# CGLemon/Sayuri

Measured on AMD Instinct MI355X. Metric: nn_evals_per_sec, higher is better.
Workload: dtype f16

## Files before the change

sayuri_amd/csrc/hip/engine_graph.h:

```cpp
#pragma once
#include "engine_plan.h"

namespace sayuri {

class EngineBase {
public:
    virtual ~EngineBase() {}
    virtual int load_tensor(int layer, int kind, const float* host, size_t n) = 0;
    virtual int upload(int n, const float* planes, const int* board_sizes, const unsigned* packed = nullptr, int binary = 0) = 0;
    virtual int run() = 0;
    virtual int sync() = 0;
    virtual int download(float* prob, float* pass, float* misc, float* own) = 0;
    virtual int time_runs(int iters, float* ms) = 0;
    virtual int profile_run(sayuri_hip_kernel_stat* rows, int cap) = 0;
    virtual int submit(int n, const float* planes, const int* bsz, float* prob, float* pass, float* misc, float* own,
                       int* ticket, const unsigned* packed = nullptr, int binary = 0) = 0;
    virtual int wait(int ticket) = 0;
    virtual int query(int ticket) = 0;
    virtual int mark_kernel(const char* name) = 0;
    virtual int timed_stat(sayuri_hip_kernel_stat* row) = 0;
    virtual size_t device_bytes() const = 0;
    virtual int last_chains() const = 0;
    virtual int tower_state() const = 0;
    virtual int latency_state() const = 0;
// ... 1085 lines not shown
    int rows_use(const Fwd& f, const ConvParams& p, const char* layer) {
        const void* use[3] = {p.in, p.out, p.res};
        for (int u = 0; u < 3 && flags_.dbg_recycle_input < 2; ++u)
            for (int i = 0; i < kNumBufs; ++i) {
                if (!use[u] || f.io.bufs[i] != use[u]) continue;
                const int stride = u ? p.cout_s : p.cin_s;
                if (rows_stride_[i] && rows_stride_[i] != stride)
                    return fail(std::string("activation buffer ") + std::to_string(i) + " is used with row stride " + std::to_string(stride) + " by " +
                                layer + " and with " + std::to_string(rows_stride_[i]) + " by " + (rows_first_[i] ? rows_first_[i] : "?") +
                                " inside one persistent run / chained forward: the rows of different tiles would overlap");
                rows_stride_[i] = stride;
                rows_first_[i] = layer;
            }
        return 0;
    }

    const ConvLayerDev& cv(int id) const { return convs_.at(id); }
    const FcLayerDev& fc(int id) const { return fcs_.at(id); }

    int forward(int t, float* zc_pass = nullptr, float* zc_misc = nullptr) {
        const int G = chains_for_batch();
        last_chains_ = G;
        rows_reset();
        IoSlot& io = io_[t];
        Fwd f{t, io, compute_[t]};
        f.ntiles = plan().ntiles;
        f.ns = geom_.n;
        f.px = geom_.total;
        f.pass = zc_pass ? zc_pass : io.pass;
        f.misc = zc_misc ? zc_misc : io.misc;
        if (sx_kts_) {
            int nse = 0;
            for (const auto& b : blocks_) nse += b.apply_se ? 1 : 0;
            if (io.sx_epoch > 0xfff00000u) {
                HIP_OK(hipMemsetAsync(io.sx_xchg, 0, sizeof(unsigned long long) * (size_t)max_batch_ * sx_kts_ * kSxMaxSub * kSxSlots, f.stream));
                io.sx_epoch = 0;
            }
            f.sx_epoch0 = io.sx_epoch;
            io.sx_epoch += (unsigned)nse;
        }
        if (G <= 1) return forward_graph(f);
        if (chain_setup(G)) return -1;
        const BoardTabs* tabs = nullptr;
        if (board_tabs(f, &tabs)) return -1;
        HIP_OK(hipEventRecord(chain_fork_, f.stream));
        const int nt = board_plan_.ntiles;
        for (int g = 0; g < G; ++g) {
            Fwd c = f;
            c.stream = chain_stream_[g];
            c.chained = true;
            c.tile0 = (int)((long)nt * g / G);
            c.ntiles = (int)((long)nt * (g + 1) / G) - c.tile0;
            c.n0 = board_plan_.tile_first[c.tile0];
            c.ns = board_plan_.tile_first[c.tile0 + c.ntiles] - c.n0;
            c.px = geom_.off[c.n0 + c.ns] - geom_.off[c.n0];
            hipError_t e = hipStreamWaitEvent(c.stream, chain_fork_, 0);
            if (flags_.chains_serial && g > 0 && e == hipSuccess) e = hipStreamWaitEvent(c.stream, chain_join_[g - 1], 0);
            if (e == hipSuccess && forward_graph(c)) return -1;
            if (e == hipSuccess) e = hipEventRecord(chain_join_[g], c.stream);
            if (e != hipSuccess) return fail(std::string("chained forward: ") + hipGetErrorString(e));
        }
        for (int g = 0; g < G; ++g) HIP_OK(hipStreamWaitEvent(f.stream, chain_join_[g], 0));
        return 0;
    }

    int pack_input(Fwd& f, T* dst) {
        const int cin = desc_.input_channels, cs = cv(SAYURI_L_INPUT_CONV).cin_s, board = board_;
        const int n0 = f.n0, ns = f.ns;
        const double px = f.px;
        const BatchGeom g = dgeom(f.io);
        const IoSlot& io = f.io;
        if (io.packed_binary > 0) {
            const unsigned* rec = io.packed_src ? io.packed_src : io.packed;
            const int split = io.packed_src ? 1 : kPackSplit;
            const int nbin = io.packed_binary, words = nbin * 12 + 8;
            return timed(f, "pack_input", 0, (double)ns * words * 4 + px * cs * sizeof(T), [&] {
                hipLaunchKernelGGL(pack_bits_kernel<T>, dim3(ns * split), dim3(256), 0, f.stream, rec, words, nbin, dst, g, cin, cs,
                                   io.g_perm, n0, split);
            });
        }
        const int grid = ns * kPackSplit;
        const int chunk = pack_input_chunk(slot_pix_, cs, (int)sizeof(T));
        const size_t lds = (size_t)chunk * (cs * sizeof(T) + 16);
        const size_t flat_lds = pack_input_flat_lds(slot_pix_, cs, (int)sizeof(T));
        const bool flat = flat_lds <= 64 * 1024 && (size_t)cin * board * board < 65536;
        return timed(f, "pack_input", 0, px * cin * 4 + px * cs * sizeof(T), [&] {
            if (flat)
                hipLaunchKernelGGL(pack_input_flat_kernel<T>, dim3(ns), dim3(kPackFlatThreads), flat_lds, f.stream,
                                   (const float*)io.planes, dst, g, cin, cs, board, io.g_perm, n0);
            else
                hipLaunchKernelGGL(pack_input_kernel<T>, dim3(grid), dim3(kPackThreads), lds, f.stream,
                                   (const float*)io.planes, dst, g, cin, cs, board, io.g_perm, chunk, n0);
        });
    }

    int forward_graph(Fwd& f) {
        const auto& d = desc_;
        const int C = d.residual_channels, csC = round_up(C, 32), act = d.default_act;
        T* const* buf = f.io.bufs;

        int x = f.take();
        const int in = f.take();
        if (pack_input(f, buf[in])) return -1;
        if (conv(f, "conv3x3_input", cv(SAYURI_L_INPUT_CONV), buf[in], buf[x], nullptr, act)) return -1;
        if (flags_.dbg_recycle_input) f.give(in);

        for (int b = 0; b < d.residual_blocks; ++b) {
            const auto& bd = blocks_[b];
            const bool se = bd.apply_se != 0;
            const int last_act = se ? (int)kIdentity : act;
            const int y = f.take();
            int skip = x;
            bool se_done = false;
            if (bd.type == SAYURI_BLOCK_RESIDUAL) {
                const int t0 = f.take();
                if (conv(f, "conv3x3_tower", cv(SAYURI_L_BLOCK(b, SAYURI_S_CONV1)), buf[x], buf[t0], nullptr, act)) return -1;
                int fused = 1;
                if (se) {
                    fused = conv_se(f, cv(SAYURI_L_BLOCK(b, SAYURI_S_CONV2)), fc(SAYURI_L_BLOCK(b, SAYURI_S_SQUEEZE)),
                                    fc(SAYURI_L_BLOCK(b, SAYURI_S_EXCITE)), buf[t0], buf[y], buf[x], C, act);
                    if (fused == 1)
                        fused = conv_sx(f, cv(SAYURI_L_BLOCK(b, SAYURI_S_CONV2)), fc(SAYURI_L_BLOCK(b, SAYURI_S_SQUEEZE)),
                                        fc(SAYURI_L_BLOCK(b, SAYURI_S_EXCITE)), buf[t0], buf[y], buf[x], C, act);
                    if (fused < 0) return -1;
                    se_done = fused == 0;
                }
                if (fused == 1 &&
                    conv(f, "conv3x3_tower", cv(SAYURI_L_BLOCK(b, SAYURI_S_CONV2)), buf[t0], buf[y], se ? nullptr : buf[x], last_act))
                    return -1;
                f.give(t0);
            } else if (bd.type == SAYURI_BLOCK_BOTTLENECK) {
                const int t0 = f.take(), t1 = f.take();
                if (conv(f, "conv1x1_tower", cv(SAYURI_L_BLOCK(b, SAYURI_S_PRE_BTL)), buf[x], buf[t0], nullptr, act)) return -1;
                if (conv(f, "conv3x3_tower", cv(SAYURI_L_BLOCK(b, SAYURI_S_CONV1)), buf[t0], buf[t1], nullptr, act)) return -1;
                if (conv(f, "conv3x3_tower", cv(SAYURI_L_BLOCK(b, SAYURI_S_CONV2)), buf[t1], buf[t0], nullptr, act)) return -1;
                if (conv(f, "conv1x1_tower", cv(SAYURI_L_BLOCK(b, SAYURI_S_POST_BTL)), buf[t0], buf[y], se ? nullptr : buf[x], last_act)) return -1;
                f.give(t0); f.give(t1);
            } else if (bd.type == SAYURI_BLOCK_NESTED_BOTTLENECK) {
                const int r1 = f.take(), t0 = f.take(), t1 = f.take();
                if (conv(f, "conv1x1_tower", cv(SAYURI_L_BLOCK(b, SAYURI_S_PRE_BTL)), buf[x], buf[r1], nullptr, act)) return -1;
                if (conv(f, "conv3x3_tower", cv(SAYURI_L_BLOCK(b, SAYURI_S_CONV1)), buf[r1], buf[t0], nullptr, act)) return -1;
                if (conv(f, "conv3x3_tower", cv(SAYURI_L_BLOCK(b, SAYURI_S_CONV2)), buf[t0], buf[t1], buf[r1], act)) return -1;
                if (conv(f, "conv3x3_tower", cv(SAYURI_L_BLOCK(b, SAYURI_S_CONV3)), buf[t1], buf[t0], nullptr, act)) return -1;
                if (conv(f, "conv3x3_tower", cv(SAYURI_L_BLOCK(b, SAYURI_S_CONV4)), buf[t0], buf[r1], buf[t1], act)) return -1;
                if (conv(f, "conv1x1_tower", cv(SAYURI_L_BLOCK(b, SAYURI_S_POST_BTL)), buf[r1], buf[y], se ? nullptr : buf[x], last_act)) return -1;
                f.give(r1); f.give(t0); f.give(t1);
            } else {
                const int s2 = f.take(), t1 = f.take();
                if (depthwise(f, "depthwise", cv(SAYURI_L_BLOCK(b, SAYURI_S_DW_CONV)), buf[x], buf[s2], buf[x], act)) return -1;
                if (conv(f, "conv1x1_tower", cv(SAYURI_L_BLOCK(b, SAYURI_S_CONV1)), buf[s2], buf[t1], nullptr, act)) return -1;
                if (conv(f, "conv1x1_tower", cv(SAYURI_L_BLOCK(b, SAYURI_S_CONV2)), buf[t1], buf[y], se ? nullptr : buf[s2], last_act)) return -1;
                f.give(t1);
                f.give(x);
                x = s2;
                skip = s2;
            }
            if (se && !se_done) {
                if (se_unit(f, fc(SAYURI_L_BLOCK(b, SAYURI_S_SQUEEZE)), fc(SAYURI_L_BLOCK(b, SAYURI_S_EXCITE)), buf[y], buf[skip], C, csC,
                            act, f.n0, f.ns))
                    return -1;
            }
            f.give(x);
            x = y;
        }
        return heads(f, x);
    }

    int heads(Fwd& f, int x) {
        const auto& d = desc_;
        const int C = d.residual_channels, csC = round_up(C, 32), act = d.default_act;
        const int Cp = d.policy_head_channels, Cv = d.value_head_channels;
        T* const* buf = f.io.bufs;
// ... 198 lines not shown
```

sayuri_amd/csrc/hip/engine_plan.h:

```cpp
#pragma once
namespace sayuri {

static thread_local std::string g_err;
static std::atomic<unsigned> g_host_free_gen{0};
static thread_local int g_test_conv_kind = 0;
static int fail(const std::string& m) { g_err = m; return -1; }

#define HIP_OK(expr)                                                                      \
    do {                                                                                  \
        hipError_t e_ = (expr);                                                           \
        if (e_ != hipSuccess) {                                                           \
            g_err = std::string(#expr) + ": " + hipGetErrorString(e_);                    \
            return -1;                                                                    \
        }                                                                                 \
    } while (0)

static inline int round_up(int v, int m) { return (v + m - 1) / m * m; }
constexpr size_t kMaxLds = 160 * 1024;
constexpr int kNumCU = 256;

template <typename T> struct ConvKernelTable {
    typedef void (*Fn)(const ConvParams);
    struct Entry { int wmt, wnt; Fn fn; size_t (*lds)(int); int npos_cap; };
    static std::vector<Entry>& entries() {
// ... 28 lines not shown
struct GldsEntry {
    int wmt, wnt;
    void (*fn)(const GldsParams);
    void (*setup)(BatchGeom, int*, int2*);
    size_t lds;
    int npos_cap, npos, pt;
};
static std::vector<GldsEntry>& glds_entries() {
    static std::vector<GldsEntry> e;
    return e;
}
template <int WMT, int WNT> static void register_glds() {
    typedef GldsCfg<WMT, WNT> Cfg;
    glds_entries().push_back({WMT, WNT, &conv_glds_kernel<WMT, WNT>, &tile_setup_kernel<Cfg::PT, Cfg::NPOS>, Cfg::lds_bytes(),
                              Cfg::NPOS_CAP, Cfg::NPOS, Cfg::PT});
}
static void register_all_glds() {
    if (!glds_entries().empty()) return;
    register_glds<8, 3>(); register_glds<8, 2>(); register_glds<8, 1>();
    register_glds<4, 3>(); register_glds<4, 2>(); register_glds<4, 1>();
}
template <typename T> static std::vector<T> board_row_order(const std::vector<T>& img, int ko_pad, int row = 8) {
    std::vector<T> out(img.size());
    const size_t planes = img.size() / ((size_t)ko_pad * row);
    for (size_t pl = 0; pl < planes; ++pl)
        for (int r = 0; r < ko_pad; ++r)
            std::copy_n(img.begin() + (pl * ko_pad + board_row_channel(r)) * row, row, out.begin() + (pl * ko_pad + r) * row);
    return out;
}
static bool board_uses_row_order(int kot) { return (kot / 64) % 2 == 0; }
typedef void (*BoardFn)(const BoardParams);
typedef void (*BoardSeFn)(const BoardSeParams);
struct BoardEntry { int kot; BoardFn fn; BoardSeFn fn_se; size_t (*lds)(int); };
static const BoardEntry kBoardEntries[] = {
    {256, &conv_board_kernel<4>, &conv_board_se_kernel<4>, &BoardCfg<4>::lds_bytes},
    {192, &conv_board_kernel<3>, nullptr, &BoardCfg<3>::lds_bytes},
    {128, &conv_board_kernel<2>, &conv_board_se_kernel<2>, &BoardCfg<2>::lds_bytes},
};
typedef void (*SplitFn)(const SplitParams);
struct SplitEntry { int nj; SplitFn fn; };
static const SplitEntry kSplitEntries[] = {
    {1, &conv_split_kernel<1>}, {2, &conv_split_kernel<2>}, {3, &conv_split_kernel<3>}, {6, &conv_split_kernel<6>}, {12, &conv_split_kernel<12>},
};
typedef void (*HeadFn)(const HeadBoardParams);
struct HeadEntry { int rt, depth; HeadFn fn; };
static const HeadEntry kHeadEntries[] = {
    {2, 5, &head_board_kernel<2, 5>}, {4, 5, &head_board_kernel<4, 5>}, {4, 3, &head_board_kernel<4, 3>},
    {6, 3, &head_board_kernel<6, 3>}, {6, 2, &head_board_kernel<6, 2>},
};
static void enable_big_lds_glds() {
    register_all_glds();
    for (const auto& e : glds_entries())
        (void)hipFuncSetAttribute((const void*)e.fn, hipFuncAttributeMaxDynamicSharedMemorySize, (int)kMaxLds);
    (void)hipFuncSetAttribute((const void*)&conv_board_kernel<4, true>, hipFuncAttributeMaxDynamicSharedMemorySize, (int)kMaxLds);
    for (const auto& e : kHeadEntries) (void)hipFuncSetAttribute((const void*)e.fn, hipFuncAttributeMaxDynamicSharedMemorySize, (int)kMaxLds);
    (void)hipFuncSetAttribute((const void*)&conv_board_sx_kernel<2>, hipFuncAttributeMaxDynamicSharedMemorySize, (int)kMaxLds);
    for (const auto& e : kSplitEntries) (void)hipFuncSetAttribute((const void*)e.fn, hipFuncAttributeMaxDynamicSharedMemorySize, (int)kMaxLds);
    for (const auto& e : kBoardEntries) {
        (void)hipFuncSetAttribute((const void*)e.fn, hipFuncAttributeMaxDynamicSharedMemorySize, (int)kMaxLds);
        if (e.fn_se) (void)hipFuncSetAttribute((const void*)e.fn_se, hipFuncAttributeMaxDynamicSharedMemorySize, (int)kMaxLds);
    }
}
struct ConvOverride {
    bool v0 = false, no_board = false;
    int wnt = 0;
};
struct EngineFlags {
    ConvOverride conv;
    bool tower = true, se_fused = true, heads_fused = true, arith = true;
    bool latency = false;
    int latency_split = 0;
    bool tower_chain = true;
    bool tower_gen_epi = true;
    bool se_split = true;
    int tower_noepi_after = -1;
    unsigned dbg_sx_epoch0 = 0;
    bool dbg_sx_stall = false;
    int sx_dbg = 0;
    int dbg_recycle_input = 0;
    int chains = 0;
    bool chains_serial = false;
    bool tower_sync = false;
    bool fwdstat = false;
    int board_kot = 0;
    int act_override = -1;
    int board_dbg = 0, heads_dbg = 0;
    static bool off(const char* name) { const char* e = getenv(name); return e && atoi(e) == 0; }
    static EngineFlags from_env() {
        EngineFlags f;
        if (const char* e = getenv("SAYURI_CONV")) {
            if (!strncmp(e, "v0", 2)) { f.conv.v0 = true; f.conv.no_board = true; }
            else if (!strncmp(e, "glds", 4)) { f.conv.no_board = true; (void)sscanf(e, "glds:%d", &f.conv.wnt); }
        }
        f.tower = !off("SAYURI_TOWER");
        f.tower_chain = !off("SAYURI_TOWER_CHAIN");
        f.tower_gen_epi = !off("SAYURI_TOWER_GEN_EPI");
        if (const char* e = getenv("SAYURI_DEBUG_RECYCLE_INPUT")) f.dbg_recycle_input = atoi(e);
        f.se_split = !off("SAYURI_SE_SPLIT");
        if (const char* e = getenv("SAYURI_SX_DBG")) f.sx_dbg = atoi(e);
        f.dbg_sx_stall = getenv("SAYURI_DEBUG_SX_STALL") != nullptr;
        if (const char* e = getenv("SAYURI_DEBUG_SX_EPOCH0")) f.dbg_sx_epoch0 = (unsigned)strtoul(e, nullptr, 0);
        if (const char* e = getenv("SAYURI_TOWER_NOEPI_AFTER")) f.tower_noepi_after = atoi(e);
        f.se_fused = !off("SAYURI_SE_FUSED");
        f.heads_fused = !off("SAYURI_HEADS_FUSED");
        f.arith = !getenv("SAYURI_NO_ARITH");
        if (const char* e = getenv("SAYURI_CHAINS")) f.chains = std::max(0, std::min(atoi(e), 4));
        f.chains_serial = getenv("SAYURI_CHAINS_SERIAL") != nullptr;
        f.tower_sync = getenv("SAYURI_TOWER_SYNC") != nullptr;
        f.fwdstat = getenv("SAYURI_HIP_FWDSTAT") != nullptr;
        if (const char* e = getenv("SAYURI_LATENCY_SPLIT")) f.latency_split = std::max(0, atoi(e));
#ifdef SAYURI_EXPERIMENTS
        if (const char* e = getenv("SAYURI_BOARD_KOT")) f.board_kot = atoi(e);
        if (const char* e = getenv("SAYURI_ACT_OVERRIDE")) f.act_override = atoi(e);
        if (const char* e = getenv("SAYURI_BOARD_DBG")) f.board_dbg = atoi(e);
        if (getenv("SAYURI_HEADS_DBG")) f.heads_dbg = 1;
        if (f.board_dbg || f.heads_dbg || f.act_override >= 0) f.tower = false;
#endif
        return f;
    }
    EngineFlags for_latency() const {
        EngineFlags f = *this;
        f.latency = true;
        f.tower = false; f.se_fused = false; f.se_split = false; f.chains = 1;
        return f;
    }
};

template <typename T> static void enable_big_lds() {
    register_all_convs<T>();
    for (const auto& e : ConvKernelTable<T>::entries())
        (void)hipFuncSetAttribute((const void*)e.fn, hipFuncAttributeMaxDynamicSharedMemorySize, (int)kMaxLds);
}

static int pick_wmt(int cout_s, bool fp16) {
    const int opts16[] = {1, 2, 3, 4, 6, 8};
    const int opts32[] = {1, 2, 3, 4};
    const int* opts = fp16 ? opts16 : opts32;
    const int nopts = fp16 ? 6 : 4;
    for (int i = 0; i < nopts; ++i)
        if (opts[i] * 32 >= cout_s) return opts[i];
    int best = opts[nopts - 1], best_pad = 1 << 30;
    for (int i = nopts - 1; i >= 0; --i) {
        const int kot = opts[i] * 32, pad = round_up(cout_s, kot) - cout_s;
        if (pad < best_pad) { best_pad = pad; best = opts[i]; }
    }
    return best;
}

struct HostGeom {
    std::vector<int> bsz, off;
    int n = 0, total = 0;
    void tile_bounds(int PT, int* npos_out, int* nsub_out) const {
        int max_pos = 0, max_sub = 0;
        int s = 0;
        for (int g0 = 0; g0 < total; g0 += PT) {
            const int g1 = std::min(g0 + PT, total);
            while (s + 1 < n && off[s + 1] <= g0) ++s;
            int pos = 0, sub = 0;
            for (int m = s; m < n && off[m] < g1; ++m) {
                const int bs = bsz[m];
                const int a = std::max(g0, off[m]) - off[m], b = std::min(g1, off[m + 1]) - off[m];
                const int rows = (b - 1) / bs - a / bs + 3;
                pos += rows * (bs + 2);
                ++sub;
            }
            max_pos = std::max(max_pos, pos);
            max_sub = std::max(max_sub, sub);
        }
        *npos_out = round_up(std::max(max_pos, 16), 16);
        *nsub_out = max_sub;
    }
};

static bool tile_fits(const HostGeom& geom, int PT, int npos_cap, int* npos) {
    int nsub;
    geom.tile_bounds(PT, npos, &nsub);
    return *npos <= npos_cap && nsub <= kMaxSub;
}
static double tile_cost(const HostGeom& geom, int PT, int kot_tiles, int* ntiles) {
    *ntiles = (geom.total + PT - 1) / PT;
    return std::ceil((double)*ntiles * kot_tiles / kNumCU) * (PT + 24);
}
template <typename T> struct TileChoice { int wnt, npos, ntiles; const typename ConvKernelTable<T>::Entry* e; };
template <typename T> static bool pick_tile(const HostGeom& geom, int wmt, int kot_tiles, bool widest, TileChoice<T>* out) {
    double best = 0;
    out->e = nullptr;
    for (const auto& e : ConvKernelTable<T>::entries()) {
        int npos, ntiles;
        if (e.wmt != wmt || !tile_fits(geom, 64 * e.wnt, e.npos_cap, &npos) || e.lds(npos) > kMaxLds) continue;
        const double cost = tile_cost(geom, 64 * e.wnt, kot_tiles, &ntiles), score = widest ? -e.wnt : cost;
        if (!out->e || score < best) { best = score; *out = TileChoice<T>{e.wnt, npos, ntiles, &e}; }
    }
// ... 383 lines not shown
```

sayuri_amd/csrc/hip/head_board.h:

```cpp
#pragma once
#include "common.h"
#include "conv_board.h"
#include "small_ops.h"

namespace sayuri {

constexpr int kHeadPix = 384;

struct HeadBoardParams {
    const void* trunk;
    const void* w;
    const void* w2;
    const float* bias;
    BatchGeom g;
    int cs;
    int PT, VT;
    HeadParams h;
    unsigned long long* dbg;
    int n0;
};

__host__ __device__ inline int head_vec_floats(int rows) { return 7 * rows + 16 + (16 * rows > 1024 ? 16 * rows : 1024); }
__host__ inline bool head_board_fits(int rows, int nchunks, int depth) {
    return (size_t)nchunks * 4 * rows * 16 + (size_t)depth * 4 * kHeadPix * 16 + sizeof(float) * head_vec_floats(rows) <= 160 * 1024;
}

__device__ __forceinline__ int split_fc(const FcDev fc, const float* x, float* red, int t, int nt) {
    const int parts = max(1, min(nt / fc.out, (fc.in + 7) / 8));
    const int per = (fc.in + parts - 1) / parts;
    for (int idx = t; idx < parts * fc.out; idx += nt) {
        const int o = idx % fc.out, part = idx / fc.out;
        const int i0 = part * per, i1 = min(fc.in, i0 + per);
        const float* w = fc.wt + o;
        float a = 0.f;
        for (int i = i0; i < i1; i += 8) {
            float wv[8];
#pragma unroll
            for (int u = 0; u < 8; ++u) wv[u] = i + u < i1 ? w[(size_t)(i + u) * fc.out] : 0.f;
#pragma unroll
            for (int u = 0; u < 8; ++u) a += (i + u < i1 ? x[i + u] : 0.f) * wv[u];
        }
        red[idx] = a;
    }
    return parts;
}
__device__ __forceinline__ void fold_fc(const FcDev fc, const float* red, int parts, float* y, int act, int t, int nt) {
    for (int o = t; o < fc.out; o += nt) {
        float a = fc.b[o];
        for (int k = 0; k < parts; ++k) a += red[k * fc.out + o];
        y[o] = activate(a, act);
    }
}

template <int RT, int ACT>
__device__ __forceinline__ void head_board_tail(const HeadBoardParams& hp, unsigned char* smem, f32x4 (&acc)[RT][3], const f16x8 (&a2)[RT / 2],
                                                int wave, int lane, int n, int bs, unsigned long long* dbg) {
    constexpr int ROWS = RT * 16;
    const HeadParams& h = hp.h;
    const int tid = wave * 64 + lane, q = lane >> 4, px = lane & 15;
    const int npix = bs * bs, B2 = h.board * h.board;
    const int on_ = h.perm ? h.perm[n] : n;
    float* vec = (float*)(smem + 160 * 1024) - head_vec_floats(ROWS);
    float* pool = vec;
    float* inter = pool + 3 * ROWS;
    float* pinter = inter + 3 * ROWS;
    float* rb = pinter + ROWS;
    float* red = rb + 16;

#pragma unroll
    for (int i = 0; i < RT; ++i)
#pragma unroll
        for (int j = 0; j < 3; ++j) {
            if constexpr (ACT == kMish) {
                const f32x2 lo = mish2(f32x2{acc[i][j][0], acc[i][j][1]}), hi = mish2(f32x2{acc[i][j][2], acc[i][j][3]});
                acc[i][j] = f32x4{lo[0], lo[1], hi[0], hi[1]};
            } else {
#pragma unroll
                for (int r = 0; r < 4; ++r) acc[i][j][r] = activate(acc[i][j][r], ACT);
            }
        }
    f32x4 d[3];
#pragma unroll
    for (int j = 0; j < 3; ++j) {
        d[j] = f32x4{0.f, 0.f, 0.f, 0.f};
#pragma unroll
        for (int t = 0; t < RT / 2; ++t) {
            f16x8 b;
#pragma unroll
            for (int r = 0; r < 4; ++r) { b[r] = (f16)acc[2 * t][j][r]; b[4 + r] = (f16)acc[2 * t + 1][j][r]; }
            d[j] = __builtin_amdgcn_mfma_f32_16x16x32_f16(a2[t], b, d[j], 0, 0, 0);
        }
    }
    float* wsum = red;
    float* wmax = red + 8 * ROWS;
    bool valid[3];
#pragma unroll
    for (int j = 0; j < 3; ++j) valid[j] = (wave + 8 * j) * 16 + px < npix;
#pragma unroll
    for (int i = 0; i < RT; ++i) {
        f32x4 s4, m4;
#pragma unroll
        for (int r = 0; r < 4; ++r) {
            float a = 0.f, b = -5000.f;
#pragma unroll
            for (int j = 0; j < 3; ++j) { a += valid[j] ? acc[i][j][r] : 0.f; b = valid[j] ? fmaxf(b, acc[i][j][r]) : b; }
            a += row_ror<8>(a); b = fmaxf(b, row_ror<8>(b));
            a += row_ror<4>(a); b = fmaxf(b, row_ror<4>(b));
            a += row_ror<2>(a); b = fmaxf(b, row_ror<2>(b));
            a += row_ror<1>(a); b = fmaxf(b, row_ror<1>(b));
            s4[r] = a; m4[r] = b;
        }
        if (px == 0) {
            *(f32x4*)(wsum + wave * ROWS + i * 16 + 4 * q) = s4;
            *(f32x4*)(wmax + wave * ROWS + i * 16 + 4 * q) = m4;
        }
    }
    __syncthreads();
    if (dbg) dbg[2] = __builtin_amdgcn_s_memtime();
    float* vpool = pool + 3 * hp.PT;
    if (tid < ROWS) {
        float ss = 0.f, mm = -5000.f;
#pragma unroll
        for (int k = 0; k < 8; ++k) { ss += wsum[k * ROWS + tid]; mm = fmaxf(mm, wmax[k * ROWS + tid]); }
        const float mean = ss / (float)npix, bd = (float)bs - 14.f;
        if (tid < hp.PT) {
            if (tid < h.Cp) { pool[tid] = mean; pool[h.Cp + tid] = mean * (bd / 10.f); pool[2 * h.Cp + tid] = mm; }
        } else {
            const int c = tid - hp.PT;
            if (c < h.Cv) { vpool[c] = mean; vpool[h.Cv + c] = mean * (bd / 10.f); vpool[2 * h.Cv + c] = mean * (bd * bd / 100.f - 0.1f); }
        }
    }
    __syncthreads();
    if (dbg) dbg[3] = __builtin_amdgcn_s_memtime();
    const bool pol = tid < 128;
    const int t2 = pol ? tid : tid - 128, nt2 = pol ? 128 : 384;
    float* red2 = pol ? red : red + 256;
    float* vinter = inter + 3 * hp.PT;
    const FcDev f1 = pol ? h.p_inter : h.v_inter;
    const int parts = split_fc(f1, pol ? pool : vpool, red2, t2, nt2);
    __syncthreads();
    fold_fc(f1, red2, parts, pol ? pinter : vinter, h.act, t2, nt2);
    __syncthreads();
    if (dbg) dbg[4] = __builtin_amdgcn_s_memtime();
    const FcDev f2 = pol ? h.pass_fc : h.v_misc;
    const int parts2 = split_fc(f2, pol ? pinter : vinter, red2, t2, nt2);
    if (wave == 7) {
        const int k = lane >> 3, part = lane & 7;
        float a = 0.f;
        if (k < h.prob_ch)
            for (int c = part; c < h.Cp; c += 8) a += h.prob_w[k * h.Cp + c] * pinter[c];
        a += __shfl_xor(a, 1);
        a += __shfl_xor(a, 2);
        a += __shfl_xor(a, 4);
        if (part == 0) rb[k] = k < h.prob_ch ? a + h.prob_b[k] : 0.f;
        if (lane == 0) rb[h.prob_ch] = h.own_b[0];
    }
    __syncthreads();
    fold_fc(f2, red2, parts2, pol ? h.pass + (size_t)on_ * f2.out : h.misc + (size_t)on_ * f2.out, kIdentity, t2, nt2);
    if (dbg) dbg[5] = __builtin_amdgcn_s_memtime();
    if (q * 4 <= h.prob_ch) {
        const f32x4 rb4 = *(const f32x4*)(rb + 4 * q);
#pragma unroll
        for (int j = 0; j < 3; ++j) {
            const int p = (wave + 8 * j) * 16 + px;
            if (p >= npix) continue;
            const int y = p / bs, cell = y * h.board + (p - y * bs);
#pragma unroll
            for (int r = 0; r < 4; ++r) {
                const int row = 4 * q + r;
                const float v = d[j][r] + rb4[r];
                if (row < h.prob_ch) h.prob[((size_t)on_ * h.prob_ch + row) * B2 + cell] = v;
                else if (row == h.prob_ch) h.own[(size_t)on_ * B2 + cell] = v;
            }
        }
    }
    if (bs < h.board)
        for (int cell = tid; cell < B2; cell += 512) {
            const int y = cell / h.board, x = cell - y * h.board;
            if (y < bs && x < bs) continue;
            for (int k = 0; k < h.prob_ch; ++k) h.prob[((size_t)on_ * h.prob_ch + k) * B2 + cell] = 0.f;
            h.own[(size_t)on_ * B2 + cell] = 0.f;
        }
}

template <int RT, int DEPTH>
__global__ __launch_bounds__(512) void head_board_kernel(const HeadBoardParams hp) {
    extern __shared__ __attribute__((aligned(16))) unsigned char smem[];
    constexpr int ROWS = RT * 16;
    const int tid = threadIdx.x, lane = tid & 63;
    const int wave = __builtin_amdgcn_readfirstlane(tid >> 6);
    const int n = hp.n0 + blockIdx.x;
    const int bs = hp.g.bsz[n], npix = bs * bs;
    const int nchunks = hp.cs / kChunk;

    const uint32_t a_lds = (uint32_t)(uintptr_t)smem;
    const int a_bytes = nchunks * 4 * ROWS * 16;
    const uint32_t b_lds = a_lds + a_bytes;
    constexpr int B_BYTES = 4 * kHeadPix * 16;

    unsigned long long* dbg = hp.dbg && n < 4 && tid == 0 ? hp.dbg + n * 8 : nullptr;
    if (dbg) dbg[0] = __builtin_amdgcn_s_memtime();
    const unsigned char* gx = (const unsigned char*)hp.trunk + (size_t)n * hp.g.slot_pix * hp.cs * 2;
    const int a_instr = a_bytes / 1024;
    for (int q = wave; q < a_instr; q += 8) glds16_s(lane * 16, (const unsigned char*)hp.w + (size_t)q * 1024, a_lds + q * 1024);
    uint32_t boff[3];
#pragma unroll
    for (int i = 0; i < 3; ++i) {
        const int q = wave + 8 * i, kgq = q & 3, blk = q >> 2;
        const int p = blk * 64 + lane;
        boff[i] = (uint32_t)((p < npix ? p : 0) * hp.cs * 2 + kgq * 16);
    }
    auto issue_b = [&](int chunk) {
        const int slot = chunk % DEPTH;
#pragma unroll
        for (int i = 0; i < 3; ++i) {
            const int q = wave + 8 * i;
            glds16_s(boff[i], gx + chunk * (kChunk * 2), b_lds + slot * B_BYTES + ((q & 3) * kHeadPix + (q >> 2) * 64) * 16);
        }
    };
    for (int c = 0; c < DEPTH - 1 && c < nchunks; ++c) issue_b(c);

    const int kg = lane >> 4;
    f16x8 a2[RT / 2];
#pragma unroll
    for (int t = 0; t < RT / 2; ++t) a2[t] = *(const f16x8*)((const unsigned char*)hp.w2 + ((t * 4 + kg) * 16 + (lane & 15)) * 16);
    f32x4 acc[RT][3];
#pragma unroll
    for (int i = 0; i < RT; ++i) {
        const f32x4 b4 = *(const f32x4*)(hp.bias + i * 16 + 4 * kg);
#pragma unroll
        for (int j = 0; j < 3; ++j) acc[i][j] = b4;
    }
    for (int chunk = 0; chunk < nchunks; ++chunk) {
        if (chunk + DEPTH - 2 < nchunks) asm volatile("s_waitcnt vmcnt(%0)" ::"n"(3 * (DEPTH - 2)) : "memory");
        else asm volatile("s_waitcnt vmcnt(0)" ::: "memory");
        __builtin_amdgcn_s_barrier();
        if (chunk + DEPTH - 1 < nchunks) issue_b(chunk + DEPTH - 1);
        const unsigned char* A = smem + (size_t)(chunk * 4 + kg) * ROWS * 16 + (lane & 15) * 16;
        const unsigned char* Bc = smem + a_bytes + (chunk % DEPTH) * B_BYTES + (size_t)kg * kHeadPix * 16 + (lane & 15) * 16;
        f16x8 bf[3];
#pragma unroll
        for (int j = 0; j < 3; ++j) bf[j] = *(const f16x8*)(Bc + (wave + 8 * j) * 256);
#pragma unroll
        for (int i = 0; i < RT; ++i) {
            const f16x8 af = *(const f16x8*)(A + i * 256);
#pragma unroll
            for (int j = 0; j < 3; ++j) acc[i][j] = __builtin_amdgcn_mfma_f32_16x16x32_f16(af, bf[j], acc[i][j], 0, 0, 0);
        }
    }
    if (dbg) dbg[1] = __builtin_amdgcn_s_memtime();
    switch (hp.h.act) {
    case kMish: head_board_tail<RT, kMish>(hp, smem, acc, a2, wave, lane, n, bs, dbg); break;
    case kReLU: head_board_tail<RT, kReLU>(hp, smem, acc, a2, wave, lane, n, bs, dbg); break;
    case kIdentity: head_board_tail<RT, kIdentity>(hp, smem, acc, a2, wave, lane, n, bs, dbg); break;
    case kSwish: head_board_tail<RT, kSwish>(hp, smem, acc, a2, wave, lane, n, bs, dbg); break;
    case kELU: head_board_tail<RT, kELU>(hp, smem, acc, a2, wave, lane, n, bs, dbg); break;
    case kSELU: head_board_tail<RT, kSELU>(hp, smem, acc, a2, wave, lane, n, bs, dbg); break;
    case kGELU: head_board_tail<RT, kGELU>(hp, smem, acc, a2, wave, lane, n, bs, dbg); break;
    default: head_board_tail<RT, kHardSwish>(hp, smem, acc, a2, wave, lane, n, bs, dbg); break;
    }
    if (dbg) {
        asm volatile("s_waitcnt vmcnt(0)" ::: "memory");
        dbg[6] = __builtin_amdgcn_s_memtime();
    }
}

}
```

sayuri_amd/csrc/hip/small_ops.h:

```cpp
#pragma once
#include <algorithm>

#include "common.h"

namespace sayuri {

constexpr int kPackThreads = 128;
constexpr int kPackSplit = 4;
template <typename T>
__global__ __launch_bounds__(kPackThreads) void pack_input_kernel(const float* __restrict__ planes, T* __restrict__ out,
                                                                  BatchGeom g, int cin, int cs, int board, const int* __restrict__ perm,
                                                                  int chunk, int n0 = 0) {
    constexpr int EPP = ElemTraits<T>::kPieceElems;
    extern __shared__ __attribute__((aligned(16))) unsigned char pk_smem[];
    const int n = n0 + blockIdx.x / kPackSplit, part = blockIdx.x % kPackSplit, tid = threadIdx.x;
    const int bs = g.bsz[n], npix = bs * bs, ppr = cs / EPP, stride = cs * (int)sizeof(T) + 16;
    const int per = (npix + kPackSplit - 1) / kPackSplit, pbeg = part * per, pend = min(npix, pbeg + per);
    const size_t B2 = (size_t)board * board;
    const float* src = planes + (size_t)(perm ? perm[n] : n) * cin * B2;
    T* dst = out + (size_t)n * g.slot_pix * cs;
    for (int p0 = pbeg; p0 < pend; p0 += chunk) {
        const int np = min(chunk, pend - p0);
        if (p0 != pbeg) __syncthreads();
        for (int q = tid; q < np; q += kPackThreads) {
            const int pp = p0 + q, y = pp / bs, x = pp - y * bs;
            const float* s0 = src + y * board + x;
            for (int pb = 0; pb < ppr; pb += 6) {
                float f[6 * EPP];
#pragma unroll
                for (int k = 0; k < 6 * EPP; ++k) {
                    const int c = pb * EPP + k;
                    f[k] = c < cin ? s0[(size_t)c * B2] : 0.f;
                }
#pragma unroll
                for (int j = 0; j < 6; ++j) {
                    if (pb + j < ppr) {
                        T v[EPP];
#pragma unroll
                        for (int e = 0; e < EPP; ++e) v[e] = from_float<T>(f[j * EPP + e]);
                        *(uint4*)(pk_smem + (size_t)q * stride + (pb + j) * 16) = *(uint4*)v;
                    }
                }
            }
        }
        __syncthreads();
        for (int it = tid; it < np * ppr; it += kPackThreads) {
            const int q = it / ppr, piece = it - q * ppr;
            *(uint4*)(dst + ((size_t)p0 * ppr + it) * EPP) = *(const uint4*)(pk_smem + (size_t)q * stride + piece * 16);
        }
    }
}
constexpr int kPackFlatThreads = 512;
constexpr int kPackFlatLoads = 32;
template <typename T>
__global__ __launch_bounds__(kPackFlatThreads) void pack_input_flat_kernel(const float* __restrict__ planes, T* __restrict__ out,
                                                                            BatchGeom g, int cin, int cs, int board,
                                                                            const int* __restrict__ perm, int n0 = 0) {
    constexpr int EPP = ElemTraits<T>::kPieceElems;
    extern __shared__ __attribute__((aligned(16))) unsigned char pk_smem[];
    const int n = n0 + blockIdx.x, tid = threadIdx.x;
    const int bs = g.bsz[n], npix = bs * bs, ppr = cs / EPP, stride = cs * (int)sizeof(T) + 16;
    const int B2 = board * board, total = cin * B2;
    const float* src = planes + (size_t)(perm ? perm[n] : n) * total;
    T* dst = out + (size_t)n * g.slot_pix * cs;
    const float r_b2 = 1.0f / (float)B2, r_b = 1.0f / (float)board;
    for (int base = 0; base < total; base += kPackFlatThreads * kPackFlatLoads) {
        float f[kPackFlatLoads];
#pragma unroll
        for (int k = 0; k < kPackFlatLoads; ++k) {
            const int e = base + k * kPackFlatThreads + tid;
            f[k] = e < total ? src[e] : 0.f;
        }
#pragma unroll
        for (int k = 0; k < kPackFlatLoads; ++k) {
            const int e = base + k * kPackFlatThreads + tid;
            const int c = (int)(((float)e + 0.5f) * r_b2), r = e - c * B2;
            const int y = (int)(((float)r + 0.5f) * r_b), x = r - y * board;
            if (e < total && y < bs && x < bs) *(T*)(pk_smem + (size_t)(y * bs + x) * stride + c * (int)sizeof(T)) = from_float<T>(f[k]);
        }
    }
    __syncthreads();
    for (int it = tid; it < npix * ppr; it += kPackFlatThreads) {
        const int q = it / ppr, piece = it - q * ppr;
        T v[EPP];
        *(uint4*)v = *(const uint4*)(pk_smem + (size_t)q * stride + piece * 16);
#pragma unroll
        for (int e = 0; e < EPP; ++e)
            if (piece * EPP + e >= cin) v[e] = from_float<T>(0.f);
        *(uint4*)(dst + (size_t)it * EPP) = *(uint4*)v;
    }
}
static inline size_t pack_input_flat_lds(int slot_pix, int cs, int elem) { return (size_t)slot_pix * (cs * elem + 16); }

static inline int pack_input_chunk(int slot_pix, int cs, int elem) {
    return std::min((slot_pix + kPackSplit - 1) / kPackSplit, (64 * 1024) / (cs * elem + 16));
}

__global__ __launch_bounds__(256) void geom_stage_kernel(const int* __restrict__ stage, int max_batch, int n, int* __restrict__ off,
                                                         int* __restrict__ bsz, int* __restrict__ perm) {
    for (int i = threadIdx.x; i <= n; i += blockDim.x) off[i] = stage[i];
    for (int i = threadIdx.x; i < n; i += blockDim.x) {
        bsz[i] = stage[max_batch + 1 + i];
        perm[i] = stage[2 * max_batch + 1 + i];
    }
}

template <typename T>
__global__ __launch_bounds__(256) void pack_bits_kernel(const unsigned* __restrict__ records, int rec_words, int nbin,
                                                        T* __restrict__ out, BatchGeom g, int cin, int cs,
                                                        const int* __restrict__ perm, int n0 = 0, int split = kPackSplit) {
    constexpr int EPP = ElemTraits<T>::kPieceElems;
    __shared__ unsigned rec[40 * 13 + 8];
    const int n = n0 + blockIdx.x / split, part = blockIdx.x % split, tid = threadIdx.x;
    const int bs = g.bsz[n], npix = bs * bs, ppr = cs / EPP;
    const int per = (npix + split - 1) / split, pbeg = part * per, pend = min(npix, pbeg + per);
    const unsigned* src = records + (size_t)(perm ? perm[n] : n) * rec_words;
    for (int i = tid; i < rec_words; i += 256) rec[i < nbin * 12 ? (i / 12) * 13 + i % 12 : nbin * 13 + (i - nbin * 12)] = src[i];
    __syncthreads();
    T* dst = out + (size_t)n * g.slot_pix * cs;
    for (int it = pbeg * ppr + tid; it < pend * ppr; it += 256) {
        const int pp = it / ppr, piece = it - pp * ppr;
        const int word = pp >> 5, sh = pp & 31;
        T v[EPP];
#pragma unroll
        for (int e = 0; e < EPP; ++e) {
            const int c = piece * EPP + e;
            float f = 0.f;
            if (c < nbin) f = (float)((rec[c * 13 + word] >> sh) & 1u);
            else if (c < cin) f = __uint_as_float(rec[nbin * 13 + (c - nbin)]);
            v[e] = from_float<T>(f);
        }
        *(uint4*)(dst + (size_t)it * EPP) = *(uint4*)v;
    }
}

struct FcDev {
    const float* wt;
    const float* b;
    int in, out;
};

__device__ __forceinline__ void block_fc(const FcDev fc, const float* x, float* y, int act, int tid, int nt) {
    for (int o = tid; o < fc.out; o += nt) {
        float s0 = 0.f, s1 = 0.f;
        const float* w = fc.wt + o;
        int i = 0;
        for (; i + 8 <= fc.in; i += 8) {
            float wv[8];
#pragma unroll
            for (int u = 0; u < 8; ++u) wv[u] = w[(size_t)(i + u) * fc.out];
#pragma unroll
            for (int u = 0; u < 8; u += 2) { s0 += x[i + u] * wv[u]; s1 += x[i + u + 1] * wv[u + 1]; }
        }
        for (; i < fc.in; ++i) s0 += x[i] * w[(size_t)i * fc.out];
        y[o] = activate(fc.b[o] + (s0 + s1), act);
    }
}

template <typename T>
__device__ __forceinline__ void block_pool(const T* __restrict__ x, int npix, int C, int cs, int bs,
                                           bool value_head, float* pool, float* scratch, int tid, int nt) {
// ... 301 lines not shown
```

Before: 74770.

## Split flat input packing across row blocks and prefetch head FC weights early

The flat input-pack kernel now launches several blocks per position, each handling a band of board rows with fewer threads, to raise parallelism and cut per-block LDS. The head board kernel prefetches the first slices of FC weights, biases and probability weights into registers before the K loop and staggers the B-chunk issue, so tail latency overlaps the GEMM. The vmcnt waits are rewritten to handle a partially filled pipeline. This adds register pressure in the head kernel and more, smaller pack launches.

```diff
diff --git a/sayuri_amd/csrc/hip/engine_graph.h b/sayuri_amd/csrc/hip/engine_graph.h
--- a/sayuri_amd/csrc/hip/engine_graph.h
+++ b/sayuri_amd/csrc/hip/engine_graph.h
@@ -1191,12 +1191,13 @@
         const int grid = ns * kPackSplit;
         const int chunk = pack_input_chunk(slot_pix_, cs, (int)sizeof(T));
         const size_t lds = (size_t)chunk * (cs * sizeof(T) + 16);
-        const size_t flat_lds = pack_input_flat_lds(slot_pix_, cs, (int)sizeof(T));
-        const bool flat = flat_lds <= 64 * 1024 && (size_t)cin * board * board < 65536;
+        const bool flat = pack_input_flat_lds(slot_pix_, cs, (int)sizeof(T)) <= 64 * 1024 && (size_t)cin * board * board < 65536;
+        const int fsplit = std::min(flags_.pack_split > 0 ? flags_.pack_split : kPackFlatSplit, board);
+        const size_t flat_lds = pack_input_flat_lds(pack_flat_rows(board, fsplit) * board, cs, (int)sizeof(T));
         return timed(f, "pack_input", 0, px * cin * 4 + px * cs * sizeof(T), [&] {
             if (flat)
-                hipLaunchKernelGGL(pack_input_flat_kernel<T>, dim3(ns), dim3(kPackFlatThreads), flat_lds, f.stream,
-                                   (const float*)io.planes, dst, g, cin, cs, board, io.g_perm, n0);
+                hipLaunchKernelGGL(pack_input_flat_kernel<T>, dim3(ns * fsplit), dim3(kPackFlatThreads), flat_lds, f.stream,
+                                   (const float*)io.planes, dst, g, cin, cs, board, io.g_perm, n0, fsplit);
             else
                 hipLaunchKernelGGL(pack_input_kernel<T>, dim3(grid), dim3(kPackThreads), lds, f.stream,
                                    (const float*)io.planes, dst, g, cin, cs, board, io.g_perm, chunk, n0);
diff --git a/sayuri_amd/csrc/hip/engine_plan.h b/sayuri_amd/csrc/hip/engine_plan.h
--- a/sayuri_amd/csrc/hip/engine_plan.h
+++ b/sayuri_amd/csrc/hip/engine_plan.h
@@ -134,6 +134,7 @@
     bool chains_serial = false;
     bool tower_sync = false;
     bool fwdstat = false;
+    int pack_split = 0;
     int board_kot = 0;
     int act_override = -1;
     int board_dbg = 0, heads_dbg = 0;
@@ -160,6 +161,7 @@
         f.chains_serial = getenv("SAYURI_CHAINS_SERIAL") != nullptr;
         f.tower_sync = getenv("SAYURI_TOWER_SYNC") != nullptr;
         f.fwdstat = getenv("SAYURI_HIP_FWDSTAT") != nullptr;
+        if (const char* e = getenv("SAYURI_PACK_SPLIT")) f.pack_split = std::max(0, std::min(atoi(e), 8));
         if (const char* e = getenv("SAYURI_LATENCY_SPLIT")) f.latency_split = std::max(0, atoi(e));
 #ifdef SAYURI_EXPERIMENTS
         if (const char* e = getenv("SAYURI_BOARD_KOT")) f.board_kot = atoi(e);
diff --git a/sayuri_amd/csrc/hip/head_board.h b/sayuri_amd/csrc/hip/head_board.h
--- a/sayuri_amd/csrc/hip/head_board.h
+++ b/sayuri_amd/csrc/hip/head_board.h
@@ -25,15 +25,41 @@
     return (size_t)nchunks * 4 * rows * 16 + (size_t)depth * 4 * kHeadPix * 16 + sizeof(float) * head_vec_floats(rows) <= 160 * 1024;
 }
 
-__device__ __forceinline__ int split_fc(const FcDev fc, const float* x, float* red, int t, int nt) {
-    const int parts = max(1, min(nt / fc.out, (fc.in + 7) / 8));
+template <int PF> struct FcSlice {
+    float w[PF];
+    float b;
+};
+__device__ __forceinline__ int fc_parts(const FcDev fc, int nt) { return max(1, min(nt / fc.out, (fc.in + 7) / 8)); }
+template <int PF> __device__ __forceinline__ void fc_prefetch(const FcDev fc, int t, int nt, FcSlice<PF>& s) {
+    const int parts = fc_parts(fc, nt), per = (fc.in + parts - 1) / parts;
+    const int o = t % fc.out, part = t / fc.out;
+    const int i0 = part * per, i1 = t < parts * fc.out ? min(fc.in, i0 + per) : i0;
+    const float* w = fc.wt + o;
+#pragma unroll
+    for (int u = 0; u < PF; ++u) s.w[u] = i0 + u < i1 ? w[(size_t)(i0 + u) * fc.out] : 0.f;
+    s.b = t < fc.out ? fc.b[t] : 0.f;
+}
+template <int PF>
+__device__ __forceinline__ int split_fc(const FcDev fc, const float* x, float* red, int t, int nt, const FcSlice<PF>& pre) {
+    const int parts = fc_parts(fc, nt);
     const int per = (fc.in + parts - 1) / parts;
     for (int idx = t; idx < parts * fc.out; idx += nt) {
         const int o = idx % fc.out, part = idx / fc.out;
         const int i0 = part * per, i1 = min(fc.in, i0 + per);
         const float* w = fc.wt + o;
         float a = 0.f;
-        for (int i = i0; i < i1; i += 8) {
+        int i = i0;
+        if (idx == t) {
+#pragma unroll
+            for (int v = 0; v < PF; v += 8) {
+                if (i < i1) {
+#pragma unroll
+                    for (int u = 0; u < 8; ++u) a += (i + u < i1 ? x[i + u] : 0.f) * pre.w[v + u];
+                    i += 8;
+                }
+            }
+        }
+        for (; i < i1; i += 8) {
             float wv[8];
 #pragma unroll
             for (int u = 0; u < 8; ++u) wv[u] = i + u < i1 ? w[(size_t)(i + u) * fc.out] : 0.f;
@@ -44,17 +70,44 @@
     }
     return parts;
 }
-__device__ __forceinline__ void fold_fc(const FcDev fc, const float* red, int parts, float* y, int act, int t, int nt) {
+template <int PF>
+__device__ __forceinline__ void fold_fc(const FcDev fc, const float* red, int parts, float* y, int act, int t, int nt, const FcSlice<PF>& pre) {
     for (int o = t; o < fc.out; o += nt) {
-        float a = fc.b[o];
+        float a = o == t ? pre.b : fc.b[o];
         for (int k = 0; k < parts; ++k) a += red[k * fc.out + o];
         y[o] = activate(a, act);
     }
 }
 
+constexpr int kFcPre1 = 24, kFcPre2 = 8, kProbPre = 8;
+struct HeadTailPre {
+    FcSlice<kFcPre1> f1;
+    FcSlice<kFcPre2> f2;
+    float pw[kProbPre];
+    float pb, ob;
+};
+__device__ __forceinline__ void head_tail_prefetch(const HeadParams& h, int tid, int wave, int lane, HeadTailPre& pre) {
+    const bool pol = tid < 128;
+    const int t2 = pol ? tid : tid - 128, nt2 = pol ? 128 : 384;
+    fc_prefetch(pol ? h.p_inter : h.v_inter, t2, nt2, pre.f1);
+    fc_prefetch(pol ? h.pass_fc : h.v_misc, t2, nt2, pre.f2);
+#pragma unroll
+    for (int u = 0; u < kProbPre; ++u) pre.pw[u] = 0.f;
+    pre.pb = pre.ob = 0.f;
+    if (wave == 7) {
+        const int k = lane >> 3, part = lane & 7;
+        if (k < h.prob_ch) {
+#pragma unroll
+            for (int u = 0; u < kProbPre; ++u) pre.pw[u] = part + 8 * u < h.Cp ? h.prob_w[k * h.Cp + part + 8 * u] : 0.f;
+            pre.pb = h.prob_b[k];
+        }
+        pre.ob = h.own_b[0];
+    }
+}
+
 template <int RT, int ACT>
 __device__ __forceinline__ void head_board_tail(const HeadBoardParams& hp, unsigned char* smem, f32x4 (&acc)[RT][3], const f16x8 (&a2)[RT / 2],
-                                                int wave, int lane, int n, int bs, unsigned long long* dbg) {
+                                                const HeadTailPre& pre, int wave, int lane, int n, int bs, unsigned long long* dbg) {
     constexpr int ROWS = RT * 16;
     const HeadParams& h = hp.h;
     const int tid = wave * 64 + lane, q = lane >> 4, px = lane & 15;
@@ -137,26 +190,31 @@
     float* red2 = pol ? red : red + 256;
     float* vinter = inter + 3 * hp.PT;
     const FcDev f1 = pol ? h.p_inter : h.v_inter;
-    const int parts = split_fc(f1, pol ? pool : vpool, red2, t2, nt2);
-    __syncthreads();
-    fold_fc(f1, red2, parts, pol ? pinter : vinter, h.act, t2, nt2);
+    const int parts = split_fc(f1, pol ? pool : vpool, red2, t2, nt2, pre.f1);
+    __syncthreads();
+    fold_fc(f1, red2, parts, pol ? pinter : vinter, h.act, t2, nt2, pre.f1);
     __syncthreads();
     if (dbg) dbg[4] = __builtin_amdgcn_s_memtime();
     const FcDev f2 = pol ? h.pass_fc : h.v_misc;
-    const int parts2 = split_fc(f2, pol ? pinter : vinter, red2, t2, nt2);
+    const int parts2 = split_fc(f2, pol ? pinter : vinter, red2, t2, nt2, pre.f2);
     if (wave == 7) {
         const int k = lane >> 3, part = lane & 7;
         float a = 0.f;
-        if (k < h.prob_ch)
-            for (int c = part; c < h.Cp; c += 8) a += h.prob_w[k * h.Cp + c] * pinter[c];
+        if (k < h.prob_ch) {
+            int c = part;
+#pragma unroll
+            for (int u = 0; u < kProbPre; ++u, c += 8)
+                if (c < h.Cp) a += pre.pw[u] * pinter[c];
+            for (; c < h.Cp; c += 8) a += h.prob_w[k * h.Cp + c] * pinter[c];
+        }
         a += __shfl_xor(a, 1);
         a += __shfl_xor(a, 2);
         a += __shfl_xor(a, 4);
-        if (part == 0) rb[k] = k < h.prob_ch ? a + h.prob_b[k] : 0.f;
-        if (lane == 0) rb[h.prob_ch] = h.own_b[0];
-    }
-    __syncthreads();
-    fold_fc(f2, red2, parts2, pol ? h.pass + (size_t)on_ * f2.out : h.misc + (size_t)on_ * f2.out, kIdentity, t2, nt2);
+        if (part == 0) rb[k] = k < h.prob_ch ? a + pre.pb : 0.f;
+        if (lane == 0) rb[h.prob_ch] = pre.ob;
+    }
+    __syncthreads();
+    fold_fc(f2, red2, parts2, pol ? h.pass + (size_t)on_ * f2.out : h.misc + (size_t)on_ * f2.out, kIdentity, t2, nt2, pre.f2);
     if (dbg) dbg[5] = __builtin_amdgcn_s_memtime();
     if (q * 4 <= h.prob_ch) {
         const f32x4 rb4 = *(const f32x4*)(rb + 4 * q);
@@ -218,8 +276,8 @@
             glds16_s(boff[i], gx + chunk * (kChunk * 2), b_lds + slot * B_BYTES + ((q & 3) * kHeadPix + (q >> 2) * 64) * 16);
         }
     };
-    for (int c = 0; c < DEPTH - 1 && c < nchunks; ++c) issue_b(c);
-
+    static_assert(DEPTH >= 2 && DEPTH <= 5, "the waits of the K loop are written out for up to three chunks behind the current one");
+    issue_b(0);
     const int kg = lane >> 4;
     f16x8 a2[RT / 2];
 #pragma unroll
@@ -231,8 +289,14 @@
 #pragma unroll
         for (int j = 0; j < 3; ++j) acc[i][j] = b4;
     }
+    HeadTailPre pre;
+    head_tail_prefetch(hp.h, tid, wave, lane, pre);
+    for (int c = 1; c < DEPTH - 1 && c < nchunks; ++c) issue_b(c);
     for (int chunk = 0; chunk < nchunks; ++chunk) {
-        if (chunk + DEPTH - 2 < nchunks) asm volatile("s_waitcnt vmcnt(%0)" ::"n"(3 * (DEPTH - 2)) : "memory");
+        const int behind = min(nchunks - 1 - chunk, DEPTH - 2);
+        if (behind >= 3) asm volatile("s_waitcnt vmcnt(9)" ::: "memory");
+        else if (behind == 2) asm volatile("s_waitcnt vmcnt(6)" ::: "memory");
+        else if (behind == 1) asm volatile("s_waitcnt vmcnt(3)" ::: "memory");
         else asm volatile("s_waitcnt vmcnt(0)" ::: "memory");
         __builtin_amdgcn_s_barrier();
         if (chunk + DEPTH - 1 < nchunks) issue_b(chunk + DEPTH - 1);
@@ -250,14 +314,14 @@
     }
     if (dbg) dbg[1] = __builtin_amdgcn_s_memtime();
     switch (hp.h.act) {
-    case kMish: head_board_tail<RT, kMish>(hp, smem, acc, a2, wave, lane, n, bs, dbg); break;
-    case kReLU: head_board_tail<RT, kReLU>(hp, smem, acc, a2, wave, lane, n, bs, dbg); break;
-    case kIdentity: head_board_tail<RT, kIdentity>(hp, smem, acc, a2, wave, lane, n, bs, dbg); break;
-    case kSwish: head_board_tail<RT, kSwish>(hp, smem, acc, a2, wave, lane, n, bs, dbg); break;
-    case kELU: head_board_tail<RT, kELU>(hp, smem, acc, a2, wave, lane, n, bs, dbg); break;
-    case kSELU: head_board_tail<RT, kSELU>(hp, smem, acc, a2, wave, lane, n, bs, dbg); break;
-    case kGELU: head_board_tail<RT, kGELU>(hp, smem, acc, a2, wave, lane, n, bs, dbg); break;
-    default: head_board_tail<RT, kHardSwish>(hp, smem, acc, a2, wave, lane, n, bs, dbg); break;
+    case kMish: head_board_tail<RT, kMish>(hp, smem, acc, a2, pre, wave, lane, n, bs, dbg); break;
+    case kReLU: head_board_tail<RT, kReLU>(hp, smem, acc, a2, pre, wave, lane, n, bs, dbg); break;
+    case kIdentity: head_board_tail<RT, kIdentity>(hp, smem, acc, a2, pre, wave, lane, n, bs, dbg); break;
+    case kSwish: head_board_tail<RT, kSwish>(hp, smem, acc, a2, pre, wave, lane, n, bs, dbg); break;
+    case kELU: head_board_tail<RT, kELU>(hp, smem, acc, a2, pre, wave, lane, n, bs, dbg); break;
+    case kSELU: head_board_tail<RT, kSELU>(hp, smem, acc, a2, pre, wave, lane, n, bs, dbg); break;
+    case kGELU: head_board_tail<RT, kGELU>(hp, smem, acc, a2, pre, wave, lane, n, bs, dbg); break;
+    default: head_board_tail<RT, kHardSwish>(hp, smem, acc, a2, pre, wave, lane, n, bs, dbg); break;
     }
     if (dbg) {
         asm volatile("s_waitcnt vmcnt(0)" ::: "memory");
diff --git a/sayuri_amd/csrc/hip/small_ops.h b/sayuri_amd/csrc/hip/small_ops.h
--- a/sayuri_amd/csrc/hip/small_ops.h
+++ b/sayuri_amd/csrc/hip/small_ops.h
@@ -50,33 +50,38 @@
         }
     }
 }
-constexpr int kPackFlatThreads = 512;
-constexpr int kPackFlatLoads = 32;
+constexpr int kPackFlatThreads = 256;
+constexpr int kPackFlatLoads = 16;
+constexpr int kPackFlatSplit = 4;
+static inline int pack_flat_rows(int board, int split) { return (board + split - 1) / split; }
 template <typename T>
 __global__ __launch_bounds__(kPackFlatThreads) void pack_input_flat_kernel(const float* __restrict__ planes, T* __restrict__ out,
                                                                             BatchGeom g, int cin, int cs, int board,
-                                                                            const int* __restrict__ perm, int n0 = 0) {
+                                                                            const int* __restrict__ perm, int n0, int split) {
     constexpr int EPP = ElemTraits<T>::kPieceElems;
     extern __shared__ __attribute__((aligned(16))) unsigned char pk_smem[];
-    const int n = n0 + blockIdx.x, tid = threadIdx.x;
-    const int bs = g.bsz[n], npix = bs * bs, ppr = cs / EPP, stride = cs * (int)sizeof(T) + 16;
-    const int B2 = board * board, total = cin * B2;
-    const float* src = planes + (size_t)(perm ? perm[n] : n) * total;
-    T* dst = out + (size_t)n * g.slot_pix * cs;
-    const float r_b2 = 1.0f / (float)B2, r_b = 1.0f / (float)board;
+    const int n = n0 + blockIdx.x / split, part = blockIdx.x % split, tid = threadIdx.x;
+    const int bs = g.bsz[n], ppr = cs / EPP, stride = cs * (int)sizeof(T) + 16;
+    const int rpp = (bs + split - 1) / split, y0 = part * rpp, y1 = min(bs, y0 + rpp);
+    if (y0 >= y1) return;
+    const int B2 = board * board, span = (y1 - y0) * board, total = cin * span, npix = (y1 - y0) * bs;
+    const float* src = planes + (size_t)(perm ? perm[n] : n) * cin * B2 + y0 * board;
+    T* dst = out + ((size_t)n * g.slot_pix + y0 * bs) * cs;
+    const float r_span = 1.0f / (float)span, r_b = 1.0f / (float)board;
     for (int base = 0; base < total; base += kPackFlatThreads * kPackFlatLoads) {
         float f[kPackFlatLoads];
 #pragma unroll
         for (int k = 0; k < kPackFlatLoads; ++k) {
             const int e = base + k * kPackFlatThreads + tid;
-            f[k] = e < total ? src[e] : 0.f;
+            const int c = (int)(((float)e + 0.5f) * r_span), r = e - c * span;
+            f[k] = e < total ? src[c * B2 + r] : 0.f;
         }
 #pragma unroll
         for (int k = 0; k < kPackFlatLoads; ++k) {
             const int e = base + k * kPackFlatThreads + tid;
-            const int c = (int)(((float)e + 0.5f) * r_b2), r = e - c * B2;
+            const int c = (int)(((float)e + 0.5f) * r_span), r = e - c * span;
             const int y = (int)(((float)r + 0.5f) * r_b), x = r - y * board;
-            if (e < total && y < bs && x < bs) *(T*)(pk_smem + (size_t)(y * bs + x) * stride + c * (int)sizeof(T)) = from_float<T>(f[k]);
+            if (e < total && x < bs) *(T*)(pk_smem + (size_t)(y * bs + x) * stride + c * (int)sizeof(T)) = from_float<T>(f[k]);
         }
     }
     __syncthreads();
```

Result: no change. 75000 (median of 4 runs) (+0.3%).
